# LinChen-65/pygcn

Hardware: AMD Instinct MI355X
Metric: SpMM GEdge/s + fwd+bwd ms/epoch, 10M-node synthetic CSR, feat_dim=256 (higher is better)
Workload: dtype f32

## Files before the change

### include/gcn_spmm.h

```cpp
#ifndef GCN_SPMM_H
#define GCN_SPMM_H

#include <stddef.h>
#include <stdint.h>

#ifdef __cplusplus
extern "C" {
#endif

#define GCN_E_BADARG   (-1)
#define GCN_E_ALIGN    (-2)
#define GCN_E_WORKSPACE (-3)
#define GCN_E_CAPACITY (-4)

#define GCN_DTYPE_F32  0
#define GCN_DTYPE_BF16 1

#define GCN_ABI_VERSION 26

#define GCN_DEFAULT_ITEM_COST   64
#define GCN_DEFAULT_LONG_THRESH 256

typedef struct gcn_csr_plan {
    int64_t n_rows;
// ... 154 lines not shown
                           size_t workspace_bytes, void *stream);
int gcn_gemm_atg256_f32_b3_colsum(const float *A, int64_t lda, const int32_t *rows_a, const float *G, int64_t ldg,
                                  const int32_t *rows_g, int64_t n_list, float *out, int64_t ldo, float *colsum_g,
                                  void *workspace, size_t workspace_bytes, void *stream);

size_t gcn_gemm_atg_bf16_workspace_bytes(int64_t n_list, int64_t K, int64_t N);
int gcn_gemm_atg_bf16(const void *A, int64_t lda, const int32_t *rows_a, const void *G, int64_t ldg,
                      const int32_t *rows_g, int64_t n_list, int64_t K, int64_t N, float *out,
                      int64_t ldo, void *workspace, size_t workspace_bytes, void *stream);

int gcn_rows_pack_count(int dtype, const void *src, int64_t ld, const int64_t *rows, int64_t m, int64_t F,
                        uint32_t *bits, int32_t *counts, void *stream);
int gcn_rows_pack_values(int dtype, const void *src, int64_t ld, const int64_t *rows, int64_t m, int64_t F,
                         const int64_t *offsets, void *vals, void *stream);
int gcn_rows_unpack(int dtype, const uint32_t *bits, const int64_t *offsets, const void *vals, int64_t m,
                    int64_t F, void *dst, int64_t ldd, void *stream);
int gcn_bits_row_counts(const uint32_t *bits, int64_t m, int64_t words, int32_t *counts, void *stream);

#define GCN_PACK512_CAPACITY 29
int gcn_rows_pack512(const float *src, int64_t ld, int64_t m, uint32_t *slots, void *stream);
int gcn_spmm_csr_packed(const gcn_csr_plan *plan, const uint32_t *slots, const float *B, int64_t ldb, float *C,
                        int64_t ldc, void *workspace, size_t workspace_bytes, void *stream);

size_t gcn_bn_workspace_bytes(int64_t n_rows, int64_t F, int dtype);
int gcn_bn_stats(int dtype, const void *z, int64_t n_rows, int64_t F, int relu, float eps, float *mean,
                 float *var, float *rstd, void *workspace, size_t workspace_bytes, void *stream);
int gcn_bn_apply(int dtype, const void *z, void *y, int64_t n_rows, int64_t F, int relu, const float *mean,
                 const float *rstd, const float *gamma, const float *beta, void *stream);
int gcn_bn_backward_sums(int dtype, const void *g, const void *z, int64_t n_rows, int64_t F, int relu, float eps,
                         const float *mean, float *sum_g, float *sum_gxhat, double *coef, void *workspace,
                         size_t workspace_bytes, void *stream);
int gcn_bn_backward_apply(int dtype, const void *g, const void *z, void *dz, int64_t n_rows, int64_t F, int relu,
                          const float *gamma, const double *coef, void *stream);

size_t gcn_bn_batched_workspace_bytes(int64_t n_rows, int64_t F, int64_t batch, int dtype);
int gcn_bn_stats_batched(int dtype, const void *z, int64_t n_rows, int64_t F, int64_t batch, int relu, float eps,
                         float *mean, float *var, float *rstd, void *workspace, size_t workspace_bytes,
                         void *stream);
int gcn_bn_apply_batched(int dtype, const void *z, void *y, int64_t n_rows, int64_t F, int64_t batch, int relu,
                         const float *mean, const float *rstd, const float *gamma, const float *beta, void *stream);
int gcn_bn_backward_sums_batched(int dtype, const void *g, const void *z, int64_t n_rows, int64_t F, int64_t batch,
                                 int relu, float eps, const float *mean, float *sum_g, float *sum_gxhat,
                                 double *coef, void *workspace, size_t workspace_bytes, void *stream);
int gcn_bn_backward_apply_batched(int dtype, const void *g, const void *z, void *dz, int64_t n_rows, int64_t F,
                                  int64_t batch, int relu, const float *gamma, const double *coef, void *stream);

// ... 77 lines not shown
```

### pygcn_amd/_native.py

```python
import ctypes
import os

import torch

_HERE = os.path.dirname(os.path.abspath(__file__))
LIB_PATH = os.environ.get("GCN_SPMM_LIB") or os.path.join(_HERE, "csrc", "libgcn_spmm.so")

GCN_ABI_VERSION = 26
GCN_REDUCE_SUM = 0
GCN_REDUCE_MAX = 1
GCN_DEFAULT_ITEM_COST = 64
GCN_DEFAULT_LONG_THRESH = 256
GCN_DTYPE_F32 = 0
GCN_DTYPE_BF16 = 1

c_i32p = ctypes.POINTER(ctypes.c_int32)
c_i64p = ctypes.POINTER(ctypes.c_int64)
c_f32p = ctypes.POINTER(ctypes.c_float)


class GcnCsrPlan(ctypes.Structure):
    _fields_ = [
        ("n_rows", ctypes.c_int64), ("n_cols", ctypes.c_int64), ("nnz", ctypes.c_int64),
        ("rowptr", ctypes.c_void_p), ("rowptr_is64", ctypes.c_int32),
# ... 54 lines not shown
    "gcn_coo_to_csr_device": (i, [p, p, p, i64, i64, i64, i, p, i, p, p, p, p, sz, p]),
    "gcn_row_normalize_device": (i, [p, i, p, i64, p]),
    "gcn_gemm_xw256_workspace_bytes": (sz, []),
    "gcn_gemm_xw256_f32": (i, [p, i64, p, i64, p, i64, i64, p, sz, p]),
    "gcn_gemm_xw256_h2_workspace_bytes": (sz, []),
    "gcn_gemm_xw256_f32_h2": (i, [p, i64, p, p, i64, p, i64, i64, p, p, gemm_ep_p, p, sz, p]),
    "gcn_gemm_xw256_b3_workspace_bytes": (sz, []),
    "gcn_gemm_xw256_f32_b3": (i, [p, i64, p, p, i64, p, i64, i64, p, gemm_ep_p, p, sz, p]),
    "gcn_gemm_xw256_f32_b3_logsoftmax": (i, [p, i64, p, i64, p, p, i64, i64, p, sz, p]),
    "gcn_gemm_bf16_workspace_bytes": (sz, [i64, i64]),
    "gcn_gemm_xw_bf16": (i, [p, i64, p, i64, p, i64, i64, i64, i64, gemm_ep_p, p, sz, p]),
    "gcn_gemm_atg256_workspace_bytes": (sz, [i64]),
    "gcn_gemm_atg256_f32": (i, [p, i64, p, p, i64, p, i64, p, p, p, i64, p, sz, p]),
    "gcn_gemm_atg256_f32_b3": (i, [p, i64, p, p, i64, p, i64, p, i64, p, sz, p]),
    "gcn_gemm_atg256_f32_b3_colsum": (i, [p, i64, p, p, i64, p, i64, p, i64, p, p, sz, p]),
    "gcn_gemm_atg_bf16_workspace_bytes": (sz, [i64, i64, i64]),
    "gcn_gemm_atg_bf16": (i, [p, i64, p, p, i64, p, i64, i64, i64, p, i64, p, sz, p]),
    "gcn_rows_pack_count": (i, [i, p, i64, p, i64, i64, p, p, p]),
    "gcn_rows_pack_values": (i, [i, p, i64, p, i64, i64, p, p, p]),
    "gcn_rows_unpack": (i, [i, p, p, p, i64, i64, p, i64, p]),
    "gcn_bits_row_counts": (i, [p, i64, i64, p, p]),
    "gcn_rows_pack512": (i, [p, i64, i64, p, p]),
    "gcn_spmm_csr_packed": (i, [plan_p, p, p, i64, p, i64, p, sz, p]),
    "gcn_bn_workspace_bytes": (sz, [i64, i64, i]),
    "gcn_bn_stats": (i, [i, p, i64, i64, i, f32, p, p, p, p, sz, p]),
    "gcn_bn_apply": (i, [i, p, p, i64, i64, i, p, p, p, p, p]),
    "gcn_bn_backward_sums": (i, [i, p, p, i64, i64, i, f32, p, p, p, p, p, sz, p]),
    "gcn_bn_backward_apply": (i, [i, p, p, p, i64, i64, i, p, p, p]),
    "gcn_bn_batched_workspace_bytes": (sz, [i64, i64, i64, i]),
    "gcn_bn_stats_batched": (i, [i, p, i64, i64, i64, i, f32, p, p, p, p, sz, p]),
    "gcn_bn_apply_batched": (i, [i, p, p, i64, i64, i64, i, p, p, p, p, p]),
    "gcn_bn_backward_sums_batched": (i, [i, p, p, i64, i64, i64, i, f32, p, p, p, p, p, sz, p]),
    "gcn_bn_backward_apply_batched": (i, [i, p, p, p, i64, i64, i64, i, p, p, p]),
    "gcn_pool_workspace_bytes": (sz, [i64, i64, i64, i]),
    "gcn_masked_colsum": (i, [i, p, p, i64, i64, i64, p, p, sz, p]),
    "gcn_masked_broadcast": (i, [i, p, p, p, i64, i64, i64, p]),
    "gcn_attn_workspace_bytes": (sz, [i64, i64, i64, i]),
    "gcn_attn_scores": (i, [i, p, p, i64, i64, i64, p, p, p, sz, p]),
    "gcn_attn_normalize": (i, [p, p, p, i64, i64, p]),
    "gcn_attn_backward": (i, [i, p, p, p, p, p, i64, i64, i64, p, sz, p]),
    "gcn_select_workspace_bytes": (sz, [i64, i64]),
    "gcn_select_kth": (i, [p, i64, i64, i64, p, p, p, sz, p]),
    "gcn_select_indices": (i, [p, i64, i64, i64, p, p, p, p, sz, p]),
    "gcn_topk_flag": (i, [p, i64, i64, p, p, p]),
    "gcn_race_keys": (i, [p, i64, i64, ctypes.c_uint64, p, p]),
    "gcn_eval_workspace_bytes": (sz, [i64, i64, i64, i64]),
# ... 71 lines not shown
```

### pygcn_amd/csrc/gcn_pack.hip

```cpp
#include <hip/hip_runtime.h>

#include <cstdint>

#include "gcn_spmm.h"
#include "gcn_internal.h"

namespace {

constexpr int kWave = 64;
constexpr int kRowsPerBlock = 4;

__device__ __forceinline__ int below(unsigned long long m)
{
    return (int)__builtin_amdgcn_mbcnt_hi((uint32_t)(m >> 32), __builtin_amdgcn_mbcnt_lo((uint32_t)m, 0u));
}

__device__ __forceinline__ uint32_t or8(uint32_t v)
{
    v |= dpp_move<0xB1>(v);
    v |= dpp_move<0x4E>(v);
    v |= dpp_move<0x141>(v);
    return v;
}

// ... 155 lines not shown
        int rank = __builtin_popcountll(mask & ((1ull << (4 * i)) - 1ull));
        uint32_t *sub = image + k * 128 + 32 * q;
        if (i < 3) sub[i] = i == 0 ? lo : i == 1 ? hi : (uint32_t)__builtin_popcountll(mask);
#pragma unroll
        for (int j = 0; j < 4; ++j) {
            if ((nib >> j) & 1u) {
                if (rank < kPack512Cap) sub[3 + rank] = x[j];
                ++rank;
            }
        }
    }
    __builtin_amdgcn_fence(__ATOMIC_RELEASE, "wavefront");
    __builtin_amdgcn_wave_barrier();
    __builtin_amdgcn_fence(__ATOMIC_ACQUIRE, "wavefront");
#pragma unroll
    for (int k = 0; k < R; ++k) {
        if (k < nr) {
            const uint2 w = *(const uint2 *)(image + k * 128 + 2 * lane);
            *(uint2 *)(slots + (r0 + k) * 128 + 2 * lane) = w;
        }
    }
}

int check(const char *who, int dtype, int64_t m, int64_t F, int64_t ld)
{
    if (dtype != GCN_DTYPE_F32 && dtype != GCN_DTYPE_BF16) return gcn_internal_fail(GCN_E_BADARG, who);
    if (m < 0 || F <= 0 || F % 32 != 0 || F > INT32_MAX || ld < F || ld % 4 != 0)
        return gcn_internal_fail(GCN_E_BADARG, who);
    return 0;
}

}

extern "C" {

int gcn_rows_pack_count(int dtype, const void *src, int64_t ld, const int64_t *rows, int64_t m, int64_t F,
                        uint32_t *bits, int32_t *counts, void *stream)
{
    if (int rc = check("gcn_rows_pack_count: bad dtype / sizes (F a multiple of 32, ld a multiple of 4)", dtype, m, F, ld))
        return rc;
    if (m == 0) return 0;
    if (src == nullptr || bits == nullptr || counts == nullptr)
        return gcn_internal_fail(GCN_E_BADARG, "gcn_rows_pack_count: NULL pointer");
    if (((uintptr_t)src) % 16 != 0) return gcn_internal_fail(GCN_E_ALIGN, "gcn_rows_pack_count: 16-byte alignment required");
    const dim3 grid((unsigned)((m + kRowsPerBlock - 1) / kRowsPerBlock)), block(kWave * kRowsPerBlock);
    hipStream_t s = (hipStream_t)stream;
// ... 36 lines not shown
    hipStream_t s = (hipStream_t)stream;
    pick_dtype(dtype, [&](auto t) {
        typedef typename decltype(t)::type T;
        hipLaunchKernelGGL(unpack_kernel<T>, grid, block, 0, s, bits, offsets, (const T *)vals, m, (int)F, (T *)dst,
                           ldd);
    });
    return launched("gcn_rows_unpack launch");
}

int gcn_rows_pack512(const float *src, int64_t ld, int64_t m, uint32_t *slots, void *stream)
{
    if (m < 0 || ld < 256 || ld % 4 != 0) return gcn_internal_fail(GCN_E_BADARG, "gcn_rows_pack512: bad sizes (256 columns, ld a multiple of 4)");
    if (m == 0) return 0;
    if (src == nullptr || slots == nullptr) return gcn_internal_fail(GCN_E_BADARG, "gcn_rows_pack512: NULL pointer");
    if ((((uintptr_t)src) | ((uintptr_t)slots)) % 16 != 0)
        return gcn_internal_fail(GCN_E_ALIGN, "gcn_rows_pack512: 16-byte alignment required");
    const int64_t blocks = (m + kPack512RowsPerBlock - 1) / kPack512RowsPerBlock;
    if (blocks > INT32_MAX) return gcn_internal_fail(GCN_E_BADARG, "gcn_rows_pack512: too many rows");
    const dim3 grid((unsigned)blocks), block(kWave * kRowsPerBlock);
    hipLaunchKernelGGL(pack512_kernel, grid, block, 0, (hipStream_t)stream, src, ld, m, slots);
    return launched("gcn_rows_pack512 launch");
}

int gcn_bits_row_counts(const uint32_t *bits, int64_t m, int64_t words, int32_t *counts, void *stream)
{
    if (m < 0 || words <= 0 || words > (1 << 20))
        return gcn_internal_fail(GCN_E_BADARG, "gcn_bits_row_counts: bad sizes");
    if (m == 0) return 0;
    if (bits == nullptr || counts == nullptr) return gcn_internal_fail(GCN_E_BADARG, "gcn_bits_row_counts: NULL pointer");
    const dim3 grid((unsigned)((m * 8 + 255) / 256)), block(256);
    hipLaunchKernelGGL(bits_count_kernel, grid, block, 0, (hipStream_t)stream, bits, m, (int)words, counts);
    return launched("gcn_bits_row_counts launch");
}

}
```

### pygcn_amd/csrc/gcn_spmm.hip

```cpp
#include <hip/hip_runtime.h>

#include <algorithm>
#include <climits>
#include <cstdint>
#include <cstdio>
#include <cstring>
#include <type_traits>

#include "gcn_spmm.h"
#include "gcn_internal.h"

namespace {

constexpr int kWave = 64;
constexpr int kWavesPerBlock = 4;
constexpr int kDefaultItemCost = GCN_DEFAULT_ITEM_COST;
constexpr int kDefaultLongThresh = GCN_DEFAULT_LONG_THRESH;

thread_local char g_err[256] = "";

int fail(int code, const char *msg)
{
    std::snprintf(g_err, sizeof(g_err), "%s", msg);
    return code;
// ... 378 lines not shown
    const int rel_end = (lane < nr) ? (int)((int64_t)rp[ra + 1 + lane] - ea) : 0;
    const int ne = readlane_i(rel_end, nr - 1);
    if (p.bias != nullptr && act) {
#pragma unroll
        for (int i = 0; i < VEC; ++i) bias[i] = p.bias[f + i];
    }
    uint32_t amax = 0u;
    wide_stream<T, VEC, D, true, FLAGS, XEPI>(p, p.col + ea, p.val + ea, ne, lane, ld_off_bytes, acc, rel_end,
                                 nr, (int64_t)ra, f, act, bias, amax);
    publish_absmax<XEPI>(p, amax);
}

typedef uint32_t u32x2 __attribute__((ext_vector_type(2)));

__device__ __forceinline__ u32x2 slot_load8(uint64_t base, uint32_t nbytes, uint32_t voff)
{
    const uint32_t lo = __builtin_amdgcn_readfirstlane((uint32_t)base);
    const uint32_t hi = __builtin_amdgcn_readfirstlane((uint32_t)(base >> 32));
    void *pb = (void *)(((uint64_t)hi << 32) | lo);
    __amdgpu_buffer_rsrc_t rsrc = __builtin_amdgcn_make_buffer_rsrc(pb, 0, nbytes, 0x00020000);
    return __builtin_amdgcn_raw_buffer_load_b64(rsrc, voff, 0, 0);
}

constexpr int kPackSlotBytes = 512;
constexpr uint32_t kPackCap = GCN_PACK512_CAPACITY;
constexpr int kStageWords = 168;
constexpr int kStageTailWords = 32;
template <int D> constexpr int stage_block_words() { return kWavesPerBlock * D * kStageWords + kStageTailWords; }

__device__ __forceinline__ void wave_sync()
{
    __builtin_amdgcn_fence(__ATOMIC_RELEASE, "wavefront");
    __builtin_amdgcn_wave_barrier();
    __builtin_amdgcn_fence(__ATOMIC_ACQUIRE, "wavefront");
}

template <int D, bool ROWS>
__device__ __forceinline__ void packed_stream(const KParams &p, uint32_t *stage, const int32_t *__restrict__ colp,
                                              const float *__restrict__ valp, int ne, int lane, float (&acc)[4],
                                              int rel_end, int nr, int64_t row0, int f, const float (&bias)[4])
{
    const int q = lane >> 4, i = lane & 15;
    const uint32_t ldb_bytes = (uint32_t)(p.ldb * 4);
    const uint32_t voff = (uint32_t)lane * 8u;
    uint32_t *const sub = stage + 42 * q + 6 * (q & 1);
    uint32_t *const mine = sub + 2 * i;
    const bool upper = i >= 8;
    const uint32_t sh = 4u * (uint32_t)(i & 7);
    const uint32_t below_lo = upper ? ~0u : (1u << sh) - 1u, below_hi = upper ? (1u << sh) - 1u : 0u;
    const bool cnt_lane = i == 1;
    int r = 0;
    int rend = ROWS ? readlane_i(rel_end, 0) : INT_MAX;
    auto emit = [&](int rr) {
        store_out<float, 4, kWave, 0>(p, row0 + rr, f, true, acc, bias);
#pragma unroll
        for (int k = 0; k < 4; ++k) acc[k] = 0.f;
    };
    auto expand = [](uint32_t nibs, const uint32_t (&v)[4], float (&x)[4]) {
        uint32_t b[4];
#pragma unroll
        for (int k = 0; k < 4; ++k) b[k] = (uint32_t)__builtin_amdgcn_sbfe((int)nibs, (uint32_t)k, 1u);
        auto sel = [](uint32_t m, uint32_t yes, uint32_t no) {
            uint32_t d;
            asm("v_bfi_b32 %0, %1, %2, %3" : "=v"(d) : "v"(m), "v"(yes), "v"(no));
            return d;
        };
        uint32_t q0 = v[0], q1 = v[1], q2 = v[2];
        x[0] = __uint_as_float(q0 & b[0]);
        q0 = sel(b[0], q1, q0); q1 = sel(b[0], q2, q1); q2 = sel(b[0], v[3], q2);
        x[1] = __uint_as_float(q0 & b[1]);
        q0 = sel(b[1], q1, q0); q1 = sel(b[1], q2, q1);
        x[2] = __uint_as_float(q0 & b[2]);
        q0 = sel(b[2], q1, q0);
// ... 10 lines not shown
        if (over) {
            const u32x4 d = row_load16((uint64_t)p.B + (uint64_t)(uint32_t)c * ldb_bytes, 1024u, (uint32_t)f * 4u);
            Elem<float, 4>::unpack(__builtin_bit_cast(f32x4, d), x);
        }
#pragma unroll
        for (int k = 0; k < 4; ++k) acc[k] = fmaf(a, x[k], acc[k]);
    };

    for (int t = 0; t < ne; t += kWave) {
        const int cnt = min(kWave, ne - t);
        int cv = 0;
        float vv = 0.f;
        if (lane < cnt) {
            cv = colp[t + lane];
            vv = valp[t + lane];
        }
        for (int k = 0; k < cnt; k += D) {
            u32x2 x[D];
            int cc[D];
#pragma unroll
            for (int j = 0; j < D; ++j) {
                const bool ok = k + j < cnt;
                cc[j] = readlane_i(cv, k + j);
                x[j] = slot_load8((uint64_t)p.packed + (uint64_t)(uint32_t)cc[j] * (uint64_t)kPackSlotBytes,
                                  ok ? (uint32_t)kPackSlotBytes : 0u, voff);
            }
            wave_sync();
            uint32_t top = 0u;
#pragma unroll
            for (int j = 0; j < D; ++j) {
                *(u32x2 *)(mine + j * kStageWords) = x[j];
                top = max(top, x[j].x);
            }
            const bool any_over = __ballot(cnt_lane && top > kPackCap) != 0ull;
            wave_sync();
            constexpr int kMaskGroup = 4, kValueGroup = 2;
            static_assert(D % kMaskGroup == 0 && kMaskGroup % kValueGroup == 0, "groups");
#pragma unroll
            for (int g0 = 0; g0 < D; g0 += kMaskGroup) {
                uint32_t nibs[kMaskGroup];
                const uint32_t *first[kMaskGroup];
                u32x2 h[kMaskGroup];
                wave_sync();
#pragma unroll
                for (int j = 0; j < kMaskGroup; ++j) h[j] = *(const u32x2 *)(sub + (g0 + j) * kStageWords);
#pragma unroll
                for (int j = 0; j < kMaskGroup; ++j) {
                    nibs[j] = (upper ? h[j].y : h[j].x) >> sh;
                    int w0 = __builtin_popcount(h[j].x & below_lo) + __builtin_popcount(h[j].y & below_hi);
                    asm("" : "+v"(w0));
                    first[j] = sub + (g0 + j) * kStageWords + 3 + w0;
                }
#pragma unroll
                for (int g = 0; g < kMaskGroup; g += kValueGroup) {
                    uint32_t v[kValueGroup][4];
                    float xs[kValueGroup][4];
                    wave_sync();
#pragma unroll
                    for (int j = 0; j < kValueGroup; ++j)
#pragma unroll
                        for (int w = 0; w < 4; ++w) v[j][w] = first[g + j][w];
#pragma unroll
                    for (int j = 0; j < kValueGroup; ++j) expand(nibs[g + j], v[j], xs[j]);
#pragma unroll
                    for (int j = 0; j < kValueGroup; ++j) {
                        const int e = g0 + g + j;
                        consume(min(t + k + e, ne - 1), xs[j],
                                any_over && __ballot(sub[e * kStageWords + 2] > kPackCap) != 0ull,
                                readlane_f(vv, k + e), cc[e]);
                    }
                }
            }
        }
    }
    if (ROWS) {
        while (r < nr) {
            emit(r);
            ++r;
        }
    }
}

template <typename IdxT, int D>
__global__ __launch_bounds__(kWave *kWavesPerBlock) __attribute__((amdgpu_waves_per_eu(7, 8)))
void spmm_wide_packed_kernel(KParams p)
{
    const int lane = threadIdx.x & (kWave - 1);
    const int item =
        blockIdx.x * kWavesPerBlock + __builtin_amdgcn_readfirstlane((int)(threadIdx.x >> 6));
    if (item >= p.n_total) return;
    const int f = 16 * (lane & 15) + 4 * (lane >> 4);
    const IdxT *__restrict__ rp = (const IdxT *)p.rowptr;
    float acc[4] = {0.f, 0.f, 0.f, 0.f}, bias[4] = {0.f, 0.f, 0.f, 0.f};
    __shared__ __attribute__((aligned(16))) uint32_t stage_all[stage_block_words<D>()];
    uint32_t *stage = stage_all + __builtin_amdgcn_readfirstlane((int)(threadIdx.x >> 6)) * (D * kStageWords);

    if (item < p.n_chunks) {
        const int row = p.chunk_row[item];
        const int64_t e0 = p.chunk_e0[item];
        const int64_t e1 = min(e0 + (int64_t)p.long_thresh, (int64_t)rp[row + 1]);
        packed_stream<D, false>(p, stage, p.col + e0, p.val + e0, (int)(e1 - e0), lane, acc, 0, 0, 0, f, bias);
        float *dst = p.partial + (int64_t)item * p.F + f;
#pragma unroll
        for (int k = 0; k < 4; ++k) dst[k] = acc[k];
        return;
    }
    const int it = item - p.n_chunks;
    const int ra = p.items[2 * it], rb = p.items[2 * it + 1];
    const int nr = rb - ra;
    const int64_t ea = (int64_t)rp[ra];
    const int rel_end = (lane < nr) ? (int)((int64_t)rp[ra + 1 + lane] - ea) : 0;
    const int ne = readlane_i(rel_end, nr - 1);
    if (p.bias != nullptr) {
#pragma unroll
        for (int k = 0; k < 4; ++k) bias[k] = p.bias[f + k];
    }
    packed_stream<D, true>(p, stage, p.col + ea, p.val + ea, ne, lane, acc, rel_end, nr, (int64_t)ra, f, bias);
}

template <typename T>
__device__ __forceinline__ const char *narrow_row_ptr(const KParams &p, int c)
{
    return c < p.b_split ? (const char *)p.B + (int64_t)c * (p.ldb * (int64_t)sizeof(T))
                         : (const char *)p.B2 + (int64_t)(c - p.b_split) * (p.ldb2 * (int64_t)sizeof(T));
}

template <typename T, int VEC, int LPR, int U>
__device__ __forceinline__ void narrow_row(const KParams &p, const int32_t *__restrict__ col,
                                           const float *__restrict__ val, int64_t e0, int64_t e1,
                                           int g, unsigned ld_off, float (&acc)[VEC],
                                           bool flags = false)
{
    typedef typename Elem<T, VEC>::Raw Raw;
    constexpr int G = kWave / LPR;
    if (flags) {
        const int lane = (int)(threadIdx.x & (kWave - 1));
        for (int64_t t = e0; t < e1; t += kWave) {
            const int cnt = (int)min((int64_t)kWave, e1 - t);
            int c = 0;
            float a = 0.f;
// ... 487 lines not shown
    const dim3 block(kWave * kWavesPerBlock);
    const bool flags = kp.bflag != nullptr || kp.csel != nullptr;
    const bool extras = kp.cflag != nullptr || kp.cabsmax != nullptr;
    const int xepi = (extras || (flags && kp.log_softmax)) ? 2 : (kp.log_softmax ? 1 : 0);
    auto go = [&](auto fl, auto x) {
        pick_index(is64, [&](auto i) {
            hipLaunchKernelGGL((spmm_wide_kernel<T, VEC, typename decltype(i)::type, D, decltype(fl)::value,
                                                 decltype(x)::value>),
                               grid, block, 0, s, kp);
        });
    };
    if (flags) pick_int<0, 2>(xepi, [&](auto x) { go(std::true_type{}, x); });
    else pick_int<0, 1, 2>(xepi, [&](auto x) { go(std::false_type{}, x); });
}

int next_pow2(int v)
{
    int p = 1;
    while (p < v) p <<= 1;
    return p;
}

template <typename T, int VECW>
int spmm_typed(const gcn_csr_plan *plan, KParams &kp, hipStream_t s)
{
    const int F = kp.F;
    const bool is64 = plan->rowptr_is64 != 0;
    const bool vec_ok = (F % VECW == 0) && (((uintptr_t)kp.B) % 16 == 0) &&
                        (((uintptr_t)kp.B2) % 16 == 0) &&
                        ((kp.ldb2 * (int64_t)sizeof(T)) % 16 == 0) &&
                        (((uintptr_t)kp.C) % 16 == 0) &&
                        ((kp.ldb * (int64_t)sizeof(T)) % 16 == 0) &&
                        ((kp.ldc * (int64_t)sizeof(T)) % 16 == 0);
    const unsigned nblk = (unsigned)((kp.n_total + kWavesPerBlock - 1) / kWavesPerBlock);
    if (kp.cskip && !(F <= kWave || (vec_ok && F / VECW <= kWave))) kp.cskip = 0;
    if (kp.log_softmax && !(F <= kWave || (vec_ok && F / VECW <= kWave)))
        return fail(GCN_E_BADARG, "gcn_spmm_csr_ep: log_softmax needs the row inside one wavefront "
                                  "(F <= 64, or 16-byte aligned operands with F/lane width <= 64)");
    if (kp.n_total > 0) {
        if (kp.packed != nullptr) {
            if constexpr (sizeof(T) == 4) {
                const dim3 grid(nblk, 1), block(kWave * kWavesPerBlock);
                pick_index(is64, [&](auto i) {
                    hipLaunchKernelGGL((spmm_wide_packed_kernel<typename decltype(i)::type, 8>), grid, block, 0, s, kp);
                });
            }
        } else if (vec_ok) {
            const int lanes = F / VECW;
            if (lanes > 32) {
                dim3 grid(nblk, (unsigned)((lanes + kWave - 1) / kWave));
                launch_wide<T, VECW>(kp, is64, grid, s);
            } else {
                dim3 grid(nblk, 1);
                launch_narrow<T, VECW>(kp, is64, next_pow2(lanes), grid, s);
            }
        } else {
            const int lpr = std::min(kWave, next_pow2(F));
            dim3 grid(nblk, (unsigned)((F + lpr - 1) / lpr));
            launch_narrow<T, 1>(kp, is64, lpr, grid, s);
        }
        if (int rc = launched("spmm launch")) return rc;
    }
    if (kp.n_long > 0) {
        hipLaunchKernelGGL((spmm_long_reduce_kernel<T>), dim3((unsigned)((kp.n_long + 3) / 4)), dim3(256), 0,
                           s, kp);
        return launched("long-row reduce launch");
    }
// ... 170 lines not shown
        long_chunk0 == nullptr)
        return fail(GCN_E_BADARG, "gcn_plan_fill_host: null output or bad n_rows");
    if (item_cost <= 0) item_cost = kDefaultItemCost;
    if (long_thresh <= 0) long_thresh = kDefaultLongThresh;
    int64_t ni = 0, nc = 0, nl = 0;
    int rc = pick_index(rowptr_is64 != 0, [&](auto i) {
        return plan_walk((const typename decltype(i)::type *)rowptr_host, n_rows, item_cost, long_thresh, items,
                         n_items, chunk_row, chunk_e0, n_chunks, long_row, long_chunk0, n_long, &ni, &nc, &nl);
    });
    if (rc) return fail(rc, "gcn_plan_fill_host: output arrays too small or rowptr not monotone");
    if (ni != n_items || nc != n_chunks || nl != n_long)
        return fail(GCN_E_CAPACITY, "gcn_plan_fill_host: sizes differ from gcn_plan_count_host");
    return 0;
}

size_t gcn_spmm_workspace_bytes(const gcn_csr_plan *plan, int64_t F)
{
    if (plan == nullptr || F <= 0 || plan->n_chunks <= 0) return 0;
    return (size_t)plan->n_chunks * (size_t)F * sizeof(float);
}

static int spmm_csr_impl(const gcn_csr_plan *plan, int dtype, const void *B, int64_t ldb, void *C,
                         int64_t ldc, int64_t F, const gcn_epilogue *ep, void *workspace,
                         size_t workspace_bytes, void *stream, const void *packed)
{
    const float *bias = ep ? ep->bias : nullptr;
    const int relu = ep ? ep->relu : 0;
    const float drop_p = ep ? ep->dropout_p : 0.f;
    if (!(drop_p >= 0.f && drop_p < 1.f))
        return fail(GCN_E_BADARG, "gcn_spmm_csr_ep: dropout_p must be in [0, 1)");
    if (plan == nullptr) return fail(GCN_E_BADARG, "gcn_spmm_csr_ep: plan is NULL");
    if (dtype != GCN_DTYPE_F32 && dtype != GCN_DTYPE_BF16)
        return fail(GCN_E_BADARG, "gcn_spmm_csr_ep: unknown dtype");
    if (plan->n_rows < 0 || plan->n_cols < 0 || plan->nnz < 0 || F < 0 || F > INT32_MAX)
        return fail(GCN_E_BADARG, "gcn_spmm_csr_ep: negative size");
    if (plan->n_rows == 0 || F == 0) return 0;
    if (C == nullptr || (B == nullptr && plan->nnz > 0 && !(ep && ep->b2 && ep->b_split == 0)))
        return fail(GCN_E_BADARG, "gcn_spmm_csr_ep: B or C is NULL");
    if (ldb < F || ldc < F) return fail(GCN_E_BADARG, "gcn_spmm_csr_ep: ldb/ldc smaller than F");
    if (ldb * 4 >= ((int64_t)1 << 32))
        return fail(GCN_E_BADARG, "gcn_spmm_csr_ep: row stride of B must be below 4 GiB");
    if (plan->rowptr == nullptr || plan->items == nullptr ||
        (plan->nnz > 0 && (plan->col == nullptr || plan->val == nullptr)))
        return fail(GCN_E_BADARG, "gcn_spmm_csr_ep: plan has NULL arrays");
    if (plan->n_chunks > 0 && (plan->chunk_row == nullptr || plan->chunk_e0 == nullptr ||
                               plan->long_row == nullptr || plan->long_chunk0 == nullptr))
        return fail(GCN_E_BADARG, "gcn_spmm_csr_ep: plan has long rows but NULL chunk arrays");
// ... 30 lines not shown
    kp.drop_row_base = ep ? ep->drop_row_base : 0;
    kp.seed_lo = ep ? (uint32_t)ep->seed : 0u;
    kp.seed_hi = ep ? (uint32_t)(ep->seed >> 32) : 0u;
    kp.seed_dev = ep ? ep->seed_dev : nullptr;
    kp.csel = ep ? ep->c_row_select : nullptr;
    kp.cabsmax = ep ? (uint32_t *)ep->c_absmax : nullptr;
    kp.cskip = (ep && ep->c_skip_zero_rows && ep->c_row_nonzero) ? 1 : 0;
    kp.B2 = ep ? ep->b2 : nullptr;
    kp.ldb2 = ep && ep->b2 ? ep->ldb2 : 0;
    kp.b_split = (ep && ep->b2) ? (int32_t)std::min<int64_t>(ep->b_split, INT32_MAX) : INT32_MAX;
    if (ep && ep->b2 && (ep->b_split < 0 || ep->ldb2 < F || ep->ldb2 * 4 >= ((int64_t)1 << 32)))
        return fail(GCN_E_BADARG, "gcn_spmm_csr_ep: bad second block of B");
    kp.bflag = ep ? ep->b_row_nonzero : nullptr;
    kp.bnnz = ep ? ep->b_nnz_rows : nullptr;
    if (kp.bflag == nullptr || kp.bnnz == nullptr) kp.bflag = nullptr, kp.bnnz = nullptr;
    kp.cflag = ep ? ep->c_row_nonzero : nullptr;
    kp.log_softmax = (ep && ep->log_softmax) ? 1 : 0;
    if (kp.log_softmax && (relu || drop_p > 0.f))
        return fail(GCN_E_BADARG, "gcn_spmm_csr_ep: log_softmax cannot be combined with relu / dropout");
    kp.n_cols = (int32_t)std::min<int64_t>(plan->n_cols, INT32_MAX);
    hipStream_t s = (hipStream_t)stream;
    return pick_dtype(dtype, [&](auto t) {
        typedef typename decltype(t)::type T;
        return spmm_typed<T, Lane<T>::V>(plan, kp, s);
    });
}

int gcn_spmm_csr_ep(const gcn_csr_plan *plan, int dtype, const void *B, int64_t ldb, void *C,
                    int64_t ldc, int64_t F, const gcn_epilogue *ep, void *workspace,
                    size_t workspace_bytes, void *stream)
{
    return spmm_csr_impl(plan, dtype, B, ldb, C, ldc, F, ep, workspace, workspace_bytes, stream, nullptr);
}

int gcn_spmm_csr_packed(const gcn_csr_plan *plan, const uint32_t *slots, const float *B, int64_t ldb, float *C,
                        int64_t ldc, void *workspace, size_t workspace_bytes, void *stream)
{
    if (slots == nullptr || B == nullptr) return fail(GCN_E_BADARG, "gcn_spmm_csr_packed: slots or B is NULL");
    if ((((uintptr_t)slots) | ((uintptr_t)B) | ((uintptr_t)C)) % 16 != 0 || ldb % 4 != 0 || ldc % 4 != 0)
        return fail(GCN_E_ALIGN, "gcn_spmm_csr_packed: 16-byte aligned slots and rows required");
    return spmm_csr_impl(plan, GCN_DTYPE_F32, B, ldb, C, ldc, 256, nullptr, workspace, workspace_bytes, stream, slots);
}

int gcn_spmm_csr(const gcn_csr_plan *plan, int dtype, const void *B, int64_t ldb, void *C,
                 int64_t ldc, int64_t F, const float *bias, int relu, void *workspace,
                 size_t workspace_bytes, void *stream)
{
    gcn_epilogue ep = {};
    ep.bias = bias;
    ep.relu = relu;
    return gcn_spmm_csr_ep(plan, dtype, B, ldb, C, ldc, F, &ep, workspace, workspace_bytes, stream);
}

int gcn_relu_dropout_backward(int dtype, const void *grad_out, const void *out, void *grad_pre,
                              int64_t n_elems, float scale, void *stream)
{
    if (dtype != GCN_DTYPE_F32 && dtype != GCN_DTYPE_BF16)
        return fail(GCN_E_BADARG, "gcn_relu_dropout_backward: unknown dtype");
    if (n_elems < 0) return fail(GCN_E_BADARG, "gcn_relu_dropout_backward: negative size");
    if (n_elems == 0) return 0;
    if (grad_out == nullptr || out == nullptr || grad_pre == nullptr)
        return fail(GCN_E_BADARG, "gcn_relu_dropout_backward: NULL pointer");
    const int64_t per = lane_elems(dtype);
    const bool vec = (n_elems % per == 0) && (((uintptr_t)grad_out | (uintptr_t)out |
// ... 193 lines not shown
```

### pygcn_amd/fused.py

```python
import os
import weakref
from types import SimpleNamespace

import torch

from .graph import CSRGraph
from . import gemm as _gemm, spmm as _spmm
from .gemm import _dense_forward, _weight_grad, gemm_xw256
from .spmm import log_softmax_fusable, pack_row_flags, spmm_csr


def _describe_rows(rs, rows):
    rs.rows_user = rows
    rs.rows_u, rs.inverse = torch.unique(rows, return_inverse=True)
    rs.n_u = int(rs.rows_u.numel())
    rs.has_duplicates = rs.n_u != rows.numel()
    rs.sorted_unique = bool(not rs.has_duplicates and (rs.n_u == 0 or bool((rows == rs.rows_u).all())))


def _list_rows2(rs, rows2):
    rs.rows2, rs.n2 = rows2, int(rows2.numel())
    rs.rows2_i32 = rows2.to(torch.int32)
    rs.rows2_padded = _gemm.padded_row_list(rows2)

# ... 96 lines not shown
    return z


_PACKED_HIDDEN = os.environ.get("PYGCN_PACKED_HIDDEN", "1") != "0"


def set_packed_hidden(enabled):
    global _PACKED_HIDDEN
    _PACKED_HIDDEN = bool(enabled)


def packed_hidden():
    return _PACKED_HIDDEN


def packed_hidden_applies(h1, w2, b2, dropout_p):
    return (_PACKED_HIDDEN and dropout_p > 0.0 and h1.dtype == torch.float32 and _gemm.gemm_scheme() == "bf16x3"
            and tuple(w2.shape) == (256, 256) and w2.dtype == torch.float32 and w2.stride(1) == 1
            and _spmm.rows_pack512_usable(h1) and h1.stride(0) < (1 << 21)
            and (b2 is None or (b2.dtype == torch.float32 and b2.is_contiguous() and b2.data_ptr() % 16 == 0)))


def _layer2_packed(graph, h1, w2, b2):
    z2 = spmm_csr(graph, packed=_spmm.rows_pack512(h1))
    return _gemm.gemm_xw256_log_softmax(z2, w2, b2)


def _forward_record(dropout_p, b1, b2):
    return SimpleNamespace(scale=_spmm.dropout_scale(dropout_p), x_bound=None, z_bound=None, h_bound=None,
                           reassoc=False, keep_bits=None,
                           bias_dtypes=(b1.dtype if b1 is not None else None, b2.dtype if b2 is not None else None))


def _gcn2_forward(ctx, x, w1, b1, w2, b2, graph, dropout_p, seed, rs=None):
    restricted = rs is not None
    a1, a2 = rs.restricted(graph) if restricted else (graph, graph)
    in_launch = {} if restricted else {"dropout_p": dropout_p, "seed": seed}
    ctx.graph = graph
    fw = ctx.fw = _forward_record(dropout_p, b1, b2)
    bounded = x.dtype == torch.float32 and _gemm.gemm_needs_bounds()
    fw.x_bound = _gemm.absmax_cached(x) if bounded else None
    fw.reassoc = bool(_gemm.layer_gemm_reassociable(x, w1, b1))
    h1 = h_bound = z = None
    if fw.reassoc:
        z = input_product(graph, x, rs)
        if bounded:
            fw.z_bound = a1.inf_norm() * fw.x_bound * 1.0001
# ... 252 lines not shown
```

### pygcn_amd/spmm.py

```python
import torch

from . import _native, tuning
from .gemm import (_dense_forward, _dense_grads, _seed_fields, _weight_grad, absmax_cached, gemm_bf16,
                   gemm_handwritten, gemm_needs_bounds, gemm_xw256, known_absmax, layer_gemm,
                   layer_gemm_reassociable, padded_row_list, remember_absmax, weight_grad_rows)
from .gemm import DenseMMFunction, gemm_keep_bits_usable, gemm_scheme, set_bound_check, set_gemm_scheme
from .graph import CSRGraph, _require_cuda, as_graph
from .tuning import MIN_ROWS, REASSOC_MAX_WIDTH_RATIO

_DTYPES = {torch.float32: _native.GCN_DTYPE_F32, torch.bfloat16: _native.GCN_DTYPE_BF16}

_timing_records = None

_poison_unwritten = False


def _maybe_poisoned(shape, dtype, device):
    if _poison_unwritten:
        return torch.full(shape, float("nan"), dtype=dtype, device=device)
    return torch.empty(shape, dtype=dtype, device=device)


def set_timing_records(records):
    global _timing_records
    _timing_records = records


class PackedRows:
    __slots__ = ("slots", "dense")

    def __init__(self, slots, dense):
        self.slots, self.dense = slots, dense


PACK512_CAPACITY = 29


def rows_pack512_usable(h):
    return (h.is_cuda and h.dim() == 2 and h.dtype == torch.float32 and h.shape[1] == 256 and h.stride(1) == 1
            and h.stride(0) % 4 == 0 and h.data_ptr() % 16 == 0)


def rows_pack512(h):
    _require_cuda(h, "h")
    if not rows_pack512_usable(h):
        raise RuntimeError(f"rows_pack512: {tuple(h.shape)} {h.dtype}: fp32 [m, 256] with 16-byte aligned rows")
    slots = torch.empty((h.shape[0], 128), dtype=torch.int32, device=h.device)
    if h.shape[0]:
        _native.launch("gcn_rows_pack512", h.device, h.data_ptr(), h.stride(0), h.shape[0], slots.data_ptr())
    return PackedRows(slots, h)


def _spmm_csr_packed(graph, packed, out, tag):
    if not isinstance(graph, CSRGraph) or not isinstance(packed, PackedRows):
        raise RuntimeError("spmm_csr: graph must be a CSRGraph and packed a PackedRows")
    B, slots = packed.dense, packed.slots
    if B.shape[0] != graph.shape[1] or B.device != graph.device or not rows_pack512_usable(B) \
            or tuple(slots.shape) != (B.shape[0], 128) or not slots.is_contiguous():
        raise RuntimeError(f"size mismatch, adj {graph.shape} x packed {tuple(B.shape)}")
    n_rows = graph.shape[0]
    if out is None:
        out = torch.empty((n_rows, 256), dtype=torch.float32, device=B.device)
    elif out.shape != (n_rows, 256) or out.dtype != torch.float32 or out.stride(1) != 1:
        raise RuntimeError("spmm_csr: bad `out`")
    if n_rows == 0:
        return out
    L = _native.lib()
    plan = graph.plan(torch.float32)
    ws_bytes = L.gcn_spmm_workspace_bytes(plan, 256)
    ws = torch.empty(ws_bytes, dtype=torch.uint8, device=B.device) if ws_bytes else None
    with torch.cuda.device(B.device):
        rec = _timing_records
        if rec is not None:
            ev0, ev1 = torch.cuda.Event(enable_timing=True), torch.cuda.Event(enable_timing=True)
            ev0.record()
        _native.launch("gcn_spmm_csr_packed", B.device, plan, slots.data_ptr(), B.data_ptr(), B.stride(0),
                       out.data_ptr(), out.stride(0), ws.data_ptr() if ws is not None else None, ws_bytes)
        if rec is not None:
            ev1.record()
            rec.append((tag, ev0, ev1, graph))
    return out


def spmm_csr(graph, B=None, bias=None, relu=False, out=None, tag="fwd", dropout_p=0.0, seed=0,
             b_hint=None, B2=None, c_flags=None, log_softmax=False, c_select=None,
             skip_zero_rows=False, row_base=0, c_absmax=None, packed=None):
    if packed is not None:
        if (B is not None or bias is not None or relu or dropout_p or b_hint is not None or B2 is not None
                or c_flags is not None or log_softmax or c_select is not None or c_absmax is not None):
            raise RuntimeError("spmm_csr: a packed operand takes the plain product only")
        return _spmm_csr_packed(graph, packed, out, tag)
    if not isinstance(graph, CSRGraph):
        raise RuntimeError("spmm_csr: graph must be a CSRGraph")
    _require_cuda(B, "dense operand")
    n_b = B.shape[0] + (B2.shape[0] if B2 is not None else 0)
    if B.dim() != 2 or n_b != graph.shape[1]:
        raise RuntimeError(f"size mismatch, adj {graph.shape} x dense {(n_b,) + tuple(B.shape[1:])}")
    if B2 is not None:
        if B2.dim() != 2 or B2.shape[1] != B.shape[1] or B2.dtype != B.dtype or B2.device != B.device:
# ... 526 lines not shown
```

Measured before the change: 8.300.

## Add 384-byte pooled sparse row slot format for layer-2 packed SpMM

Adds a 384-byte packed row format that stores 8 mask words, a header of prefix counts, and one shared value pool of up to 87 nonzeros. The SpMM kernel is templated on slot geometry so it can read this format, and layer 2 now packs into it instead of the 512-byte format. The goal is fewer bytes gathered per neighbour and a higher nonzero capacity before rows fall back to dense. It adds another pack kernel variant plus header-based offset logic in the hot loop.

```diff
diff --git a/include/gcn_spmm.h b/include/gcn_spmm.h
--- a/include/gcn_spmm.h
+++ b/include/gcn_spmm.h
@@ -200,6 +200,11 @@
 int gcn_spmm_csr_packed(const gcn_csr_plan *plan, const uint32_t *slots, const float *B, int64_t ldb, float *C,
                         int64_t ldc, void *workspace, size_t workspace_bytes, void *stream);
 
+#define GCN_PACK384_CAPACITY 87
+int gcn_rows_pack384(const float *src, int64_t ld, int64_t m, uint32_t *slots, void *stream);
+int gcn_spmm_csr_packed384(const gcn_csr_plan *plan, const uint32_t *slots, const float *B, int64_t ldb, float *C,
+                           int64_t ldc, void *workspace, size_t workspace_bytes, void *stream);
+
 size_t gcn_bn_workspace_bytes(int64_t n_rows, int64_t F, int dtype);
 int gcn_bn_stats(int dtype, const void *z, int64_t n_rows, int64_t F, int relu, float eps, float *mean,
                  float *var, float *rstd, void *workspace, size_t workspace_bytes, void *stream);
diff --git a/pygcn_amd/_native.py b/pygcn_amd/_native.py
--- a/pygcn_amd/_native.py
+++ b/pygcn_amd/_native.py
@@ -100,6 +100,8 @@
     "gcn_bits_row_counts": (i, [p, i64, i64, p, p]),
     "gcn_rows_pack512": (i, [p, i64, i64, p, p]),
     "gcn_spmm_csr_packed": (i, [plan_p, p, p, i64, p, i64, p, sz, p]),
+    "gcn_rows_pack384": (i, [p, i64, i64, p, p]),
+    "gcn_spmm_csr_packed384": (i, [plan_p, p, p, i64, p, i64, p, sz, p]),
     "gcn_bn_workspace_bytes": (sz, [i64, i64, i]),
     "gcn_bn_stats": (i, [i, p, i64, i64, i, f32, p, p, p, p, sz, p]),
     "gcn_bn_apply": (i, [i, p, p, i64, i64, i, p, p, p, p, p]),
diff --git a/pygcn_amd/csrc/gcn_pack.hip b/pygcn_amd/csrc/gcn_pack.hip
--- a/pygcn_amd/csrc/gcn_pack.hip
+++ b/pygcn_amd/csrc/gcn_pack.hip
@@ -201,6 +201,72 @@
     }
 }
 
+constexpr int kPack384Cap = GCN_PACK384_CAPACITY;
+constexpr int kPack384Words = 96;
+static_assert(9 + kPack384Cap == kPack384Words, "masks + header + pool fill the slot");
+#ifndef GCN_PACK384_ROWS_PER_WAVE
+#define GCN_PACK384_ROWS_PER_WAVE 2
+#endif
+constexpr int kPack384RowsPerWave = GCN_PACK384_ROWS_PER_WAVE;
+constexpr int kPack384RowsPerBlock = kRowsPerBlock * kPack384RowsPerWave;
+
+__global__ __launch_bounds__(kWave *kRowsPerBlock) void pack384_kernel(const float *__restrict__ src, int64_t ld,
+                                                                       int64_t m, uint32_t *__restrict__ slots)
+{
+    constexpr int R = kPack384RowsPerWave;
+    __shared__ __attribute__((aligned(16))) uint32_t image_all[kRowsPerBlock * R * kPack384Words];
+    const int lane = threadIdx.x & (kWave - 1);
+    const int wave = __builtin_amdgcn_readfirstlane((int)(threadIdx.x >> 6));
+    const int64_t r0 = ((int64_t)blockIdx.x * kRowsPerBlock + wave) * R;
+    if (r0 >= m) return;
+    const int nr = (int)(m - r0 < R ? m - r0 : R);
+    const int q = lane >> 4, i = lane & 15;
+    uint32_t *image = image_all + wave * (R * kPack384Words);
+    uint4 v[R];
+#pragma unroll
+    for (int k = 0; k < R; ++k)
+        v[k] = *(const uint4 *)(src + (r0 + (k < nr ? k : nr - 1)) * ld + 16 * i + 4 * q);
+#pragma unroll
+    for (int k = 0; k < R; ++k) {
+        const uint32_t x[4] = {v[k].x, v[k].y, v[k].z, v[k].w};
+        uint32_t nib = 0u;
+#pragma unroll
+        for (int j = 0; j < 4; ++j) nib |= (x[j] != 0u ? 1u : 0u) << j;
+        const uint32_t lo = or16(i < 8 ? nib << (4 * i) : 0u), hi = or16(i >= 8 ? nib << (4 * (i - 8)) : 0u);
+        const unsigned long long mask = ((unsigned long long)hi << 32) | lo;
+        const int cq = __builtin_popcountll(mask);
+        const uint32_t s1 = (uint32_t)__builtin_amdgcn_readlane(cq, 0);
+        const uint32_t s2 = s1 + (uint32_t)__builtin_amdgcn_readlane(cq, 16);
+        const uint32_t s3 = s2 + (uint32_t)__builtin_amdgcn_readlane(cq, 32);
+        const uint32_t total = s3 + (uint32_t)__builtin_amdgcn_readlane(cq, 48);
+        const uint32_t header = s1 | (s2 << 8) | (s3 << 16) | ((total < 255u ? total : 255u) << 24);
+        int rank = (int)(q == 0 ? 0u : q == 1 ? s1 : q == 2 ? s2 : s3)
+                   + __builtin_popcountll(mask & ((1ull << (4 * i)) - 1ull));
+        uint32_t *img = image + k * kPack384Words;
+        if (i < 2) img[2 * q + i] = i == 0 ? lo : hi;
+        if (lane == 2) img[8] = header;
+#pragma unroll
+        for (int j = 0; j < 4; ++j) {
+            if ((nib >> j) & 1u) {
+                if (rank < kPack384Cap) img[9 + rank] = x[j];
+                ++rank;
+            }
+        }
+    }
+    __builtin_amdgcn_fence(__ATOMIC_RELEASE, "wavefront");
+    __builtin_amdgcn_wave_barrier();
+    __builtin_amdgcn_fence(__ATOMIC_ACQUIRE, "wavefront");
+    if (lane < kPack384Words / 2) {
+#pragma unroll
+        for (int k = 0; k < R; ++k) {
+            if (k < nr) {
+                const uint2 w = *(const uint2 *)(image + k * kPack384Words + 2 * lane);
+                *(uint2 *)(slots + (r0 + k) * kPack384Words + 2 * lane) = w;
+            }
+        }
+    }
+}
+
 int check(const char *who, int dtype, int64_t m, int64_t F, int64_t ld)
 {
     if (dtype != GCN_DTYPE_F32 && dtype != GCN_DTYPE_BF16) return gcn_internal_fail(GCN_E_BADARG, who);
@@ -283,6 +349,20 @@
     return launched("gcn_rows_pack512 launch");
 }
 
+int gcn_rows_pack384(const float *src, int64_t ld, int64_t m, uint32_t *slots, void *stream)
+{
+    if (m < 0 || ld < 256 || ld % 4 != 0) return gcn_internal_fail(GCN_E_BADARG, "gcn_rows_pack384: bad sizes (256 columns, ld a multiple of 4)");
+    if (m == 0) return 0;
+    if (src == nullptr || slots == nullptr) return gcn_internal_fail(GCN_E_BADARG, "gcn_rows_pack384: NULL pointer");
+    if ((((uintptr_t)src) | ((uintptr_t)slots)) % 16 != 0)
+        return gcn_internal_fail(GCN_E_ALIGN, "gcn_rows_pack384: 16-byte alignment required");
+    const int64_t blocks = (m + kPack384RowsPerBlock - 1) / kPack384RowsPerBlock;
+    if (blocks > INT32_MAX) return gcn_internal_fail(GCN_E_BADARG, "gcn_rows_pack384: too many rows");
+    const dim3 grid((unsigned)blocks), block(kWave * kRowsPerBlock);
+    hipLaunchKernelGGL(pack384_kernel, grid, block, 0, (hipStream_t)stream, src, ld, m, slots);
+    return launched("gcn_rows_pack384 launch");
+}
+
 int gcn_bits_row_counts(const uint32_t *bits, int64_t m, int64_t words, int32_t *counts, void *stream)
 {
     if (m < 0 || words <= 0 || words > (1 << 20))
diff --git a/pygcn_amd/csrc/gcn_spmm.hip b/pygcn_amd/csrc/gcn_spmm.hip
--- a/pygcn_amd/csrc/gcn_spmm.hip
+++ b/pygcn_amd/csrc/gcn_spmm.hip
@@ -424,11 +424,24 @@
     return __builtin_amdgcn_raw_buffer_load_b64(rsrc, voff, 0, 0);
 }
 
-constexpr int kPackSlotBytes = 512;
-constexpr uint32_t kPackCap = GCN_PACK512_CAPACITY;
-constexpr int kStageWords = 168;
-constexpr int kStageTailWords = 32;
-template <int D> constexpr int stage_block_words() { return kWavesPerBlock * D * kStageWords + kStageTailWords; }
+template <int BYTES> struct SlotGeom;
+template <> struct SlotGeom<512> {
+    static constexpr int kBytes = 512, kLanes = 64, kStageWords = 168, kTailWords = 32;
+    static constexpr uint32_t kCap = GCN_PACK512_CAPACITY;
+    static constexpr bool kPooled = false;
+    static __device__ __forceinline__ int mask_word(int q) { return 42 * q + 6 * (q & 1); }
+    static __device__ __forceinline__ int own_word(int q, int i) { return mask_word(q) + 2 * i; }
+    static __device__ __forceinline__ int pool_word(int q) { return mask_word(q) + 3; }
+};
+template <> struct SlotGeom<384> {
+    static constexpr int kBytes = 384, kLanes = 48, kStageWords = 128, kTailWords = 9 + 252 + 4 - 128;
+    static constexpr uint32_t kCap = GCN_PACK384_CAPACITY;
+    static constexpr bool kPooled = true;
+    static __device__ __forceinline__ int mask_word(int q) { return 2 * q; }
+    static __device__ __forceinline__ int own_word(int q, int i) { return 2 * (16 * q + i); }
+    static __device__ __forceinline__ int pool_word(int) { return 9; }
+};
+template <typename G, int D> constexpr int stage_block_words() { return kWavesPerBlock * D * G::kStageWords + G::kTailWords; }
 
 __device__ __forceinline__ void wave_sync()
 {
@@ -437,7 +450,7 @@
     __builtin_amdgcn_fence(__ATOMIC_ACQUIRE, "wavefront");
 }
 
-template <int D, bool ROWS>
+template <typename G, int D, bool ROWS>
 __device__ __forceinline__ void packed_stream(const KParams &p, uint32_t *stage, const int32_t *__restrict__ colp,
                                               const float *__restrict__ valp, int ne, int lane, float (&acc)[4],
                                               int rel_end, int nr, int64_t row0, int f, const float (&bias)[4])
@@ -445,12 +458,14 @@
     const int q = lane >> 4, i = lane & 15;
     const uint32_t ldb_bytes = (uint32_t)(p.ldb * 4);
     const uint32_t voff = (uint32_t)lane * 8u;
-    uint32_t *const sub = stage + 42 * q + 6 * (q & 1);
-    uint32_t *const mine = sub + 2 * i;
+    uint32_t *const sub = stage + G::mask_word(q);
+    uint32_t *const mine = stage + G::own_word(q, i);
+    uint32_t *const pool = stage + G::pool_word(q);
     const bool upper = i >= 8;
     const uint32_t sh = 4u * (uint32_t)(i & 7);
     const uint32_t below_lo = upper ? ~0u : (1u << sh) - 1u, below_hi = upper ? (1u << sh) - 1u : 0u;
     const bool cnt_lane = i == 1;
+    const uint32_t pre_off = q > 0 ? 8u * (uint32_t)(q - 1) : 0u, pre_len = q > 0 ? 8u : 0u;
     int r = 0;
     int rend = ROWS ? readlane_i(rel_end, 0) : INT_MAX;
     auto emit = [&](int rr) {
@@ -507,17 +522,19 @@
             for (int j = 0; j < D; ++j) {
                 const bool ok = k + j < cnt;
                 cc[j] = readlane_i(cv, k + j);
-                x[j] = slot_load8((uint64_t)p.packed + (uint64_t)(uint32_t)cc[j] * (uint64_t)kPackSlotBytes,
-                                  ok ? (uint32_t)kPackSlotBytes : 0u, voff);
+                x[j] = slot_load8((uint64_t)p.packed + (uint64_t)(uint32_t)cc[j] * (uint64_t)G::kBytes,
+                                  ok ? (uint32_t)G::kBytes : 0u, voff);
             }
             wave_sync();
-            uint32_t top = 0u;
+            uint32_t top = 0u, hdr[D];
 #pragma unroll
             for (int j = 0; j < D; ++j) {
-                *(u32x2 *)(mine + j * kStageWords) = x[j];
-                top = max(top, x[j].x);
-            }
-            const bool any_over = __ballot(cnt_lane && top > kPackCap) != 0ull;
+                *(u32x2 *)(mine + j * G::kStageWords) = x[j];
+                if constexpr (G::kPooled) hdr[j] = (uint32_t)__builtin_amdgcn_readlane((int)x[j].x, 4);
+                else top = max(top, x[j].x);
+            }
+            bool any_over = true;
+            if constexpr (!G::kPooled) any_over = __ballot(cnt_lane && top > G::kCap) != 0ull;
             wave_sync();
             constexpr int kMaskGroup = 4, kValueGroup = 2;
             static_assert(D % kMaskGroup == 0 && kMaskGroup % kValueGroup == 0, "groups");
@@ -528,13 +545,22 @@
                 u32x2 h[kMaskGroup];
                 wave_sync();
 #pragma unroll
-                for (int j = 0; j < kMaskGroup; ++j) h[j] = *(const u32x2 *)(sub + (g0 + j) * kStageWords);
+                for (int j = 0; j < kMaskGroup; ++j) h[j] = *(const u32x2 *)(sub + (g0 + j) * G::kStageWords);
 #pragma unroll
                 for (int j = 0; j < kMaskGroup; ++j) {
                     nibs[j] = (upper ? h[j].y : h[j].x) >> sh;
-                    int w0 = __builtin_popcount(h[j].x & below_lo) + __builtin_popcount(h[j].y & below_hi);
+                    int w0;
+                    if constexpr (G::kPooled) {
+                        w0 = (int)__builtin_amdgcn_ubfe(hdr[g0 + j], pre_off, pre_len);
+                        asm("" : "+v"(w0));
+                        w0 += __builtin_popcount(h[j].x & below_lo);
+                        asm("" : "+v"(w0));
+                        w0 += __builtin_popcount(h[j].y & below_hi);
+                    } else {
+                        w0 = __builtin_popcount(h[j].x & below_lo) + __builtin_popcount(h[j].y & below_hi);
+                    }
                     asm("" : "+v"(w0));
-                    first[j] = sub + (g0 + j) * kStageWords + 3 + w0;
+                    first[j] = pool + (g0 + j) * G::kStageWords + w0;
                 }
 #pragma unroll
                 for (int g = 0; g < kMaskGroup; g += kValueGroup) {
@@ -550,9 +576,10 @@
 #pragma unroll
                     for (int j = 0; j < kValueGroup; ++j) {
                         const int e = g0 + g + j;
-                        consume(min(t + k + e, ne - 1), xs[j],
-                                any_over && __ballot(sub[e * kStageWords + 2] > kPackCap) != 0ull,
-                                readlane_f(vv, k + e), cc[e]);
+                        bool over;
+                        if constexpr (G::kPooled) over = hdr[e] >= ((G::kCap + 1u) << 24);
+                        else over = any_over && __ballot(sub[e * G::kStageWords + 2] > G::kCap) != 0ull;
+                        consume(min(t + k + e, ne - 1), xs[j], over, readlane_f(vv, k + e), cc[e]);
                     }
                 }
             }
@@ -566,7 +593,7 @@
     }
 }
 
-template <typename IdxT, int D>
+template <typename IdxT, int D, int SLOT>
 __global__ __launch_bounds__(kWave *kWavesPerBlock) __attribute__((amdgpu_waves_per_eu(7, 8)))
 void spmm_wide_packed_kernel(KParams p)
 {
@@ -577,14 +604,15 @@
     const int f = 16 * (lane & 15) + 4 * (lane >> 4);
     const IdxT *__restrict__ rp = (const IdxT *)p.rowptr;
     float acc[4] = {0.f, 0.f, 0.f, 0.f}, bias[4] = {0.f, 0.f, 0.f, 0.f};
-    __shared__ __attribute__((aligned(16))) uint32_t stage_all[stage_block_words<D>()];
-    uint32_t *stage = stage_all + __builtin_amdgcn_readfirstlane((int)(threadIdx.x >> 6)) * (D * kStageWords);
+    typedef SlotGeom<SLOT> G;
+    __shared__ __attribute__((aligned(16))) uint32_t stage_all[stage_block_words<G, D>()];
+    uint32_t *stage = stage_all + __builtin_amdgcn_readfirstlane((int)(threadIdx.x >> 6)) * (D * G::kStageWords);
 
     if (item < p.n_chunks) {
         const int row = p.chunk_row[item];
         const int64_t e0 = p.chunk_e0[item];
         const int64_t e1 = min(e0 + (int64_t)p.long_thresh, (int64_t)rp[row + 1]);
-        packed_stream<D, false>(p, stage, p.col + e0, p.val + e0, (int)(e1 - e0), lane, acc, 0, 0, 0, f, bias);
+        packed_stream<G, D, false>(p, stage, p.col + e0, p.val + e0, (int)(e1 - e0), lane, acc, 0, 0, 0, f, bias);
         float *dst = p.partial + (int64_t)item * p.F + f;
 #pragma unroll
         for (int k = 0; k < 4; ++k) dst[k] = acc[k];
@@ -600,7 +628,7 @@
 #pragma unroll
         for (int k = 0; k < 4; ++k) bias[k] = p.bias[f + k];
     }
-    packed_stream<D, true>(p, stage, p.col + ea, p.val + ea, ne, lane, acc, rel_end, nr, (int64_t)ra, f, bias);
+    packed_stream<G, D, true>(p, stage, p.col + ea, p.val + ea, ne, lane, acc, rel_end, nr, (int64_t)ra, f, bias);
 }
 
 template <typename T>
@@ -1134,7 +1162,7 @@
 }
 
 template <typename T, int VECW>
-int spmm_typed(const gcn_csr_plan *plan, KParams &kp, hipStream_t s)
+int spmm_typed(const gcn_csr_plan *plan, KParams &kp, hipStream_t s, int slot_bytes)
 {
     const int F = kp.F;
     const bool is64 = plan->rowptr_is64 != 0;
@@ -1153,8 +1181,11 @@
         if (kp.packed != nullptr) {
             if constexpr (sizeof(T) == 4) {
                 const dim3 grid(nblk, 1), block(kWave * kWavesPerBlock);
-                pick_index(is64, [&](auto i) {
-                    hipLaunchKernelGGL((spmm_wide_packed_kernel<typename decltype(i)::type, 8>), grid, block, 0, s, kp);
+                pick_int<512, 384>(slot_bytes, [&](auto g) {
+                    pick_index(is64, [&](auto i) {
+                        hipLaunchKernelGGL((spmm_wide_packed_kernel<typename decltype(i)::type, 8, decltype(g)::value>),
+                                           grid, block, 0, s, kp);
+                    });
                 });
             }
         } else if (vec_ok) {
@@ -1371,7 +1402,7 @@
 
 static int spmm_csr_impl(const gcn_csr_plan *plan, int dtype, const void *B, int64_t ldb, void *C,
                          int64_t ldc, int64_t F, const gcn_epilogue *ep, void *workspace,
-                         size_t workspace_bytes, void *stream, const void *packed)
+                         size_t workspace_bytes, void *stream, const void *packed, int slot_bytes = 512)
 {
     const float *bias = ep ? ep->bias : nullptr;
     const int relu = ep ? ep->relu : 0;
@@ -1448,7 +1479,7 @@
     hipStream_t s = (hipStream_t)stream;
     return pick_dtype(dtype, [&](auto t) {
         typedef typename decltype(t)::type T;
-        return spmm_typed<T, Lane<T>::V>(plan, kp, s);
+        return spmm_typed<T, Lane<T>::V>(plan, kp, s, slot_bytes);
     });
 }
 
@@ -1466,6 +1497,16 @@
     if ((((uintptr_t)slots) | ((uintptr_t)B) | ((uintptr_t)C)) % 16 != 0 || ldb % 4 != 0 || ldc % 4 != 0)
         return fail(GCN_E_ALIGN, "gcn_spmm_csr_packed: 16-byte aligned slots and rows required");
     return spmm_csr_impl(plan, GCN_DTYPE_F32, B, ldb, C, ldc, 256, nullptr, workspace, workspace_bytes, stream, slots);
+}
+
+int gcn_spmm_csr_packed384(const gcn_csr_plan *plan, const uint32_t *slots, const float *B, int64_t ldb, float *C,
+                           int64_t ldc, void *workspace, size_t workspace_bytes, void *stream)
+{
+    if (slots == nullptr || B == nullptr) return fail(GCN_E_BADARG, "gcn_spmm_csr_packed384: slots or B is NULL");
+    if ((((uintptr_t)slots) | ((uintptr_t)B) | ((uintptr_t)C)) % 16 != 0 || ldb % 4 != 0 || ldc % 4 != 0)
+        return fail(GCN_E_ALIGN, "gcn_spmm_csr_packed384: 16-byte aligned slots and rows required");
+    return spmm_csr_impl(plan, GCN_DTYPE_F32, B, ldb, C, ldc, 256, nullptr, workspace, workspace_bytes, stream, slots,
+                         384);
 }
 
 int gcn_spmm_csr(const gcn_csr_plan *plan, int dtype, const void *B, int64_t ldb, void *C,
diff --git a/pygcn_amd/fused.py b/pygcn_amd/fused.py
--- a/pygcn_amd/fused.py
+++ b/pygcn_amd/fused.py
@@ -142,7 +142,7 @@
 
 
 def _layer2_packed(graph, h1, w2, b2):
-    z2 = spmm_csr(graph, packed=_spmm.rows_pack512(h1))
+    z2 = spmm_csr(graph, packed=_spmm.rows_pack384(h1))
     return _gemm.gemm_xw256_log_softmax(z2, w2, b2)
 
 
diff --git a/pygcn_amd/spmm.py b/pygcn_amd/spmm.py
--- a/pygcn_amd/spmm.py
+++ b/pygcn_amd/spmm.py
@@ -27,13 +27,18 @@
 
 
 class PackedRows:
-    __slots__ = ("slots", "dense")
-
-    def __init__(self, slots, dense):
+    __slots__ = ("slots", "dense", "slot_bytes")
+
+    def __init__(self, slots, dense, slot_bytes=None):
         self.slots, self.dense = slots, dense
+        self.slot_bytes = 4 * slots.shape[1] if slot_bytes is None else int(slot_bytes)
+        if self.slot_bytes not in _PACKED_ENTRY:
+            raise RuntimeError(f"PackedRows: no slot format of {self.slot_bytes} bytes (512 or 384)")
 
 
 PACK512_CAPACITY = 29
+PACK384_CAPACITY = 87
+_PACKED_ENTRY = {512: "gcn_spmm_csr_packed", 384: "gcn_spmm_csr_packed384"}
 
 
 def rows_pack512_usable(h):
@@ -48,7 +53,17 @@
     slots = torch.empty((h.shape[0], 128), dtype=torch.int32, device=h.device)
     if h.shape[0]:
         _native.launch("gcn_rows_pack512", h.device, h.data_ptr(), h.stride(0), h.shape[0], slots.data_ptr())
-    return PackedRows(slots, h)
+    return PackedRows(slots, h, 512)
+
+
+def rows_pack384(h):
+    _require_cuda(h, "h")
+    if not rows_pack512_usable(h):
+        raise RuntimeError(f"rows_pack384: {tuple(h.shape)} {h.dtype}: fp32 [m, 256] with 16-byte aligned rows")
+    slots = torch.empty((h.shape[0], 96), dtype=torch.int32, device=h.device)
+    if h.shape[0]:
+        _native.launch("gcn_rows_pack384", h.device, h.data_ptr(), h.stride(0), h.shape[0], slots.data_ptr())
+    return PackedRows(slots, h, 384)
 
 
 def _spmm_csr_packed(graph, packed, out, tag):
@@ -56,7 +71,7 @@
         raise RuntimeError("spmm_csr: graph must be a CSRGraph and packed a PackedRows")
     B, slots = packed.dense, packed.slots
     if B.shape[0] != graph.shape[1] or B.device != graph.device or not rows_pack512_usable(B) \
-            or tuple(slots.shape) != (B.shape[0], 128) or not slots.is_contiguous():
+            or tuple(slots.shape) != (B.shape[0], packed.slot_bytes // 4) or not slots.is_contiguous():
         raise RuntimeError(f"size mismatch, adj {graph.shape} x packed {tuple(B.shape)}")
     n_rows = graph.shape[0]
     if out is None:
@@ -74,7 +89,7 @@
         if rec is not None:
             ev0, ev1 = torch.cuda.Event(enable_timing=True), torch.cuda.Event(enable_timing=True)
             ev0.record()
-        _native.launch("gcn_spmm_csr_packed", B.device, plan, slots.data_ptr(), B.data_ptr(), B.stride(0),
+        _native.launch(_PACKED_ENTRY[packed.slot_bytes], B.device, plan, slots.data_ptr(), B.data_ptr(), B.stride(0),
                        out.data_ptr(), out.stride(0), ws.data_ptr() if ws is not None else None, ws_bytes)
         if rec is not None:
             ev1.record()
```

New measurement: 8.592, median of 6. +3.5%, better.
